# Tencent-RoboticsX/lifelike-agility-and-play

Measured on AMD Instinct MI355X. Metric: env-steps/sec (whole node), PMC tracking env, random policy, higher is better.
Workload: dtype f32

## Files before the change

### lifelike_agility_and_play_amd/csrc/llenv.hip

```cpp
#include <hip/hip_runtime.h>

#include <stdlib.h>

#include <new>
#include <type_traits>

#include "lanes.hpp"
#include "epmc_engine.hpp"
#include "sepmc_engine.hpp"
#include "pmc_engine.hpp"
#include "pmc_step.hpp"
#include "launch_plan.hpp"

#define HIPCHK(call)                                                                                   \
  do {                                                                                                 \
    hipError_t _e = (call);                                                                            \
    if (_e != hipSuccess) throw PmcError(LL_EHIP, std::string(#call) + ": " + hipGetErrorString(_e)); \
  } while (0)

typedef Pmc<GpuLanes> K;
typedef GpuLanesPinned<LC_COUNT> GpuLanes1;
#ifndef LL_PIN_EPMC
#define LL_PIN_EPMC 0
#endif
#ifndef LL_PIN_SEPMC
#define LL_PIN_SEPMC 0
#endif
#ifndef LL_PIN_PMC
#define LL_PIN_PMC 1
#endif
#ifndef LL_CONE_LDS
#define LL_CONE_LDS 1
#endif
#ifndef LL_CONE_LDS_SEPMC
#define LL_CONE_LDS_SEPMC 1
#endif
#ifndef LL_CONE_LDS_SEPMC1
#define LL_CONE_LDS_SEPMC1 1
#endif
#ifndef LL_PARK
#define LL_PARK 1
#endif
#ifndef LL_RELOAD_PMC
#define LL_RELOAD_PMC 1
#endif
#ifndef LL_RELOAD_EPMC1
#define LL_RELOAD_EPMC1 2
#endif
#ifndef LL_RELOAD_EPMC2
#define LL_RELOAD_EPMC2 1
#endif
#ifndef LL_SEPMC_RAY_CHUNK
#define LL_SEPMC_RAY_CHUNK 3
#endif
#ifndef LL_RELOAD_SEPMC2
#define LL_RELOAD_SEPMC2 1
#endif
#ifndef LL_SEPMC_ONE_WAVE_DEFAULT
#define LL_SEPMC_ONE_WAVE_DEFAULT 1
#endif
#ifndef LL_GRAM_PIPE_PMC1
#define LL_GRAM_PIPE_PMC1 0
#endif
typedef GpuLanesPinned<LC_COUNT, LL_PIN_PMC ? 7 : 0, LL_PIN_PMC ? BC_COUNT : 0, LL_PIN_PMC ? LK_BASE : 0> GpuLanesPmc1Plain;
typedef std::conditional<LL_GRAM_PIPE_PMC1 != 0, WithGramPipe<GpuLanesPmc1Plain>, GpuLanesPmc1Plain>::type GpuLanesPmc1;

__device__ __forceinline__ double wave_sum(double x) {
  for (int d = 32; d > 0; d >>= 1) x += __shfl_xor(x, d);
  return x;
}
__device__ __forceinline__ double ld_agent(const double* p) {
  return __builtin_bit_cast(double, __hip_atomic_load(reinterpret_cast<const unsigned long long*>(p), __ATOMIC_RELAXED, __HIP_MEMORY_SCOPE_AGENT));
}
__device__ __forceinline__ void st_agent(double* p, double v) {
  __hip_atomic_store(reinterpret_cast<unsigned long long*>(p), __builtin_bit_cast(unsigned long long, v), __ATOMIC_RELAXED, __HIP_MEMORY_SCOPE_AGENT);
}
__device__ __forceinline__ const StepParams& kernarg_params() {
  const __attribute__((address_space(4))) void* k = (const __attribute__((address_space(4))) void*)__builtin_amdgcn_kernarg_segment_ptr();
  asm volatile("" : "+s"(k));
  return *(const StepParams*)(const __attribute__((address_space(4))) StepParams*)k;
}
__device__ __forceinline__ void table_fold_wave(const StepParams& P, int sl, bool last_step) {
  const int lane = threadIdx.x & 63, n = P.n_clips;
  unsigned long long* pend_r = P.pending_reward + (long)sl * n;
  unsigned long long* pend_l = P.pending_len + (long)sl * n;
  const double* prev = sl == 0 ? P.cdf : P.cdf_ver + (long)sl * n;
  double* dst = last_step ? P.cdf : P.cdf_ver + (long)(sl + 1) * n;
  bool mine = false;
  for (int c = lane; c < n; c += PMC_WAVE) {
    const unsigned long long pr = __hip_atomic_load(pend_r + c, __ATOMIC_RELAXED, __HIP_MEMORY_SCOPE_AGENT);
    const unsigned long long pl = __hip_atomic_load(pend_l + c, __ATOMIC_RELAXED, __HIP_MEMORY_SCOPE_AGENT);
    if (pr) {
      st_agent(P.avg_reward + c, (double)__uint_as_float((uint32_t)pr));
      st_agent(P.avg_len + c, (double)__uint_as_float((uint32_t)pl));
      __hip_atomic_store(pend_r + c, 0ull, __ATOMIC_RELAXED, __HIP_MEMORY_SCOPE_AGENT);
      __hip_atomic_store(pend_l + c, 0ull, __ATOMIC_RELAXED, __HIP_MEMORY_SCOPE_AGENT);
      mine = true;
    }
  }
  if (!__any(mine)) {
    if (dst != prev) for (int c = lane; c < n; c += PMC_WAVE) st_agent(dst + c, ld_agent(prev + c));
    return;
  }
  asm volatile("s_waitcnt vmcnt(0)" ::: "memory");
  double part = 0.0;
  for (int c = lane; c < n; c += PMC_WAVE) {
    const double p = pow(1.0 - ld_agent(P.avg_reward + c), P.sample_factor);
    st_agent(P.prob + c, p);
    part += p;
  }
  asm volatile("s_waitcnt vmcnt(0)" ::: "memory");
  const double inv = 1.0 / wave_sum(part);
  double carry = 0.0;
  for (int c0 = 0; c0 < n; c0 += PMC_WAVE) {
    const int c = c0 + lane;
    double x = 0.0;
    if (c < n) { x = ld_agent(P.prob + c) * inv; st_agent(P.prob + c, x); }
    for (int d = 1; d < PMC_WAVE; d <<= 1) {
      const double y = __shfl_up(x, d);
      if (lane >= d) x += y;
    }
    x += carry;
    if (c < n) st_agent(dst + c, (c == n - 1) ? 1.0 : x);
    carry = __shfl(x, PMC_WAVE - 1);
  }
}
__device__ __attribute__((noinline)) void table_fold_wave_out_of_line(const StepParams& P, int sl, bool last_step) { table_fold_wave(P, sl, last_step); }
__device__ __forceinline__ void step_done_fold(const StepParams& P, int sl, bool last_step, bool multi) {
  asm volatile("s_waitcnt vmcnt(0)" ::: "memory");
  unsigned int ticket = 0;
  if (threadIdx.x == 0) ticket = __hip_atomic_fetch_add(P.block_ticket + sl, 1u, __ATOMIC_RELAXED, __HIP_MEMORY_SCOPE_AGENT);
  ticket = __builtin_amdgcn_readfirstlane(ticket);
  if (ticket != gridDim.x - 1) return;
  if (multi && sl > 0) {
    while (__hip_atomic_load(P.ver_ready + (sl - 1), __ATOMIC_RELAXED, __HIP_MEMORY_SCOPE_AGENT) != P.launch_serial) __builtin_amdgcn_s_sleep(2);
    LL_VER_FENCE(__ATOMIC_ACQUIRE);
  }
  asm volatile("" ::: "memory");
  if (multi) table_fold_wave_out_of_line(P, sl, last_step);
  else table_fold_wave(P, sl, last_step);
  if (threadIdx.x == 0) __hip_atomic_store(P.block_ticket + sl, 0u, __ATOMIC_RELAXED, __HIP_MEMORY_SCOPE_AGENT);
  if (multi) {
    asm volatile("s_waitcnt vmcnt(0)" ::: "memory");
    LL_VER_FENCE(__ATOMIC_RELEASE);
    if (threadIdx.x == 0) {
      __hip_atomic_store(P.ver_ready + sl, P.launch_serial, __ATOMIC_RELAXED, __HIP_MEMORY_SCOPE_AGENT);
      if (last_step) __hip_atomic_store(P.resident, 0u, __ATOMIC_RELAXED, __HIP_MEMORY_SCOPE_AGENT);
    }
  }
}

__device__ __forceinline__ float4 random_action_group(const StepParams& P, uint32_t gid, float sigma, int sl = 0) {
  uint32_t r[4];
  const uint64_t step = P.step_count + (uint64_t)sl;
  philox4x32(gid, (uint32_t)step, (uint32_t)(step >> 32), 0xAC710u, (uint32_t)P.seed, (uint32_t)(P.seed >> 32), r);
  const float k = 2.3283064365386963e-10f;
  float u1 = fminf(((float)r[0] + 1.0f) * k, 1.0f), u2 = (float)r[1] * k, u3 = fminf(((float)r[2] + 1.0f) * k, 1.0f), u4 = (float)r[3] * k;
  float m1 = sqrtf(-2.0f * logf(u1)), m2 = sqrtf(-2.0f * logf(u3));
  float4 o;
  o.x = sigma * m1 * cosf(6.283185307179586f * u2); o.y = sigma * m1 * sinf(6.283185307179586f * u2);
  o.z = sigma * m2 * cosf(6.283185307179586f * u4); o.w = sigma * m2 * sinf(6.283185307179586f * u4);
  return o;
}

template <class Lanes>
__device__ __forceinline__ void step_actions(const StepParams& P, const Lanes& ln, float* lds, int env, int sl, float* act) {
  if (P.action_sigma > 0.0f) {
    float* stash = lds + LC_COUNT * 4 + CAND_TABLE_WORDS * PMC_ROW + (threadIdx.x >> 4) * 12;
    const int l16 = threadIdx.x & 15;
    const uint32_t g = (uint32_t)(l16 < 3 ? l16 : 0);
    const float4 o = random_action_group(P, (uint32_t)env * 3u + g, P.action_sigma, sl);
    if (l16 < 3) {
      reinterpret_cast<float4*>(P.actions_out)[(long)env * 3 + l16] = o;
      reinterpret_cast<float4*>(stash)[l16] = o;
    }
    asm volatile("s_waitcnt lgkmcnt(0)" ::: "memory");
    for (int j = 0; j < 3; j++) act[j] = stash[ln.leg() * 3 + j];
  } else {
    for (int j = 0; j < 3; j++) act[j] = ln.ldl(P.actions, (long)env * 12 + j, 3);
  }
}

template <int OCC, bool OBST = false, bool MULTI = false, bool CONE = false, bool XROWS = false>
__global__ __launch_bounds__(PMC_WAVE, OCC) void pmc_step_kernel(StepParams P) {
  extern __shared__ __attribute__((aligned(16))) float lds[];
  const int env0 = blockIdx.x * PMC_ENVS_PER_WAVE + (threadIdx.x >> 4);
  typedef WithParamsReload<typename std::conditional<OCC == 1, GpuLanesPmc1, GpuLanes>::type, LL_RELOAD_PMC> Lanes0;
  typedef typename std::conditional<(OCC == 2 && CONE && LL_CONE_LDS), WithConeInLds<Lanes0>, Lanes0>::type Lanes;
  Lanes ln(lds);
  if constexpr (OCC == 1) ln.stage_consts(P.legc, LC_COUNT, P.candc, CAND_TABLE_WORDS, P.basec);
  else ln.stage_consts(P.legc, LC_COUNT, P.candc, CAND_TABLE_WORDS);
  if constexpr (!MULTI) {
    if (env0 < P.n_envs) {
      float act[3];
      step_actions(P, ln, lds, env0, 0, act);
      Pmc<Lanes>::template step_env<OBST, CONE, XROWS>(ln, P, env0, act, 0);
    }
    step_done_fold(P, 0, true, false);
  } else {
    if (threadIdx.x == 0) __hip_atomic_fetch_add(P.resident, 1u, __ATOMIC_RELAXED, __HIP_MEMORY_SCOPE_AGENT);
    for (int sl = 0; sl < P.n_steps; sl++) {
      if (sl) __builtin_amdgcn_fence(__ATOMIC_SEQ_CST, "workgroup");
      ln.new_step();
      int env = env0;
      asm volatile("" : "+v"(env));
      if (env < P.n_envs) {
        float act[3];
        PMC_PHASE("step.actions");
        step_actions(P, ln, lds, env, sl, act);
        Pmc<Lanes>::template step_env<OBST, CONE, XROWS>(ln, P, env, act, sl);
      }
      PMC_PHASE("step.table_fold");
      const StepParams& Pr = kernarg_params();
      step_done_fold(Pr, sl, sl == Pr.n_steps - 1, true);
    }
  }
}

template <int OCC, bool MULTI = false, bool CONE = false, bool XROWS = false>
__global__ __launch_bounds__(PMC_WAVE, OCC) void epmc_step_kernel(StepParams P, EpmcParams E) {
  extern __shared__ __attribute__((aligned(16))) float lds[];
  const int env0 = blockIdx.x * PMC_ENVS_PER_WAVE + (threadIdx.x >> 4);
  typedef WithRayChunk<WithShapePrefetch<WithParamsReload<typename std::conditional<OCC == 1 && LL_PIN_EPMC, GpuLanes1, GpuLanes>::type, (OCC == 1 ? LL_RELOAD_EPMC1 : LL_RELOAD_EPMC2)>, OCC == 2>, (OCC == 1 ? (MULTI ? 7 : 3) : 1)> Lanes0;
  typedef typename std::conditional<(OCC == 2 && CONE && LL_CONE_LDS), WithConeInLds<Lanes0>, Lanes0>::type Lanes;
  Lanes ln(lds);
  ln.stage_consts(P.legc, LC_COUNT, P.candc, CAND_TABLE_WORDS);
  if (env0 >= P.n_envs) return;
  if constexpr (!MULTI) {
    float act[3];
    step_actions(P, ln, lds, env0, 0, act);
    Epmc<Lanes>::template step_env<((OCC == 2 && LL_PARK) || LL_PARK > 1), CONE, XROWS>(ln, P, E, env0, act);
  } else {
    for (int sl = 0; sl < P.n_steps; sl++) {
      if (sl) __builtin_amdgcn_fence(__ATOMIC_SEQ_CST, "workgroup");
      ln.new_step();
      int env = env0;
      asm volatile("" : "+v"(env));
      float act[3];
      step_actions(P, ln, lds, env, sl, act);
      Epmc<Lanes>::template step_env<(LL_PARK > 1), CONE, XROWS>(ln, P, E, env, act);
    }
  }
}
__global__ __launch_bounds__(PMC_WAVE) void epmc_reset_kernel(StepParams P, EpmcParams E, const int32_t* ids, int n, const float* draws, const float* prev_orn) {
  extern __shared__ __attribute__((aligned(16))) float lds[];
  const int i = blockIdx.x * PMC_ENVS_PER_WAVE + (threadIdx.x >> 4);
  GpuLanes ln(lds);
  ln.stage_consts(P.legc, LC_COUNT, P.candc, CAND_TABLE_WORDS);
  if (i >= n) return;
  const int env = ids ? ids[i] : i;
  Epmc<GpuLanes>::reset_env(ln, P, E, env, draws ? draws + (long)i * EPMC_MAX_DRAWS : nullptr, prev_orn ? prev_orn + (long)i * 4 : nullptr);
}

#define PERCEPT_THREADS 128
__global__ __launch_bounds__(PERCEPT_THREADS) void epmc_percept_kernel(StepParams P, EpmcParams E) {
  __shared__ __attribute__((aligned(16))) float lists[3][EPMC_MAX_BOXES * EPMC_BOX_WORDS];
  __shared__ int cnt[3];
  const int row = blockIdx.x;
  const float* rec = E.ray_pose + (long)row * EPMC_RAY_POSE;
  if (threadIdx.x < 3) cnt[threadIdx.x] = 0;
  __syncthreads();
  typedef Epmc<GpuLanes> EP;
  const int nb = (int)rec[14];
  if ((int)threadIdx.x < nb) {
    M3<float> R;
    for (int i = 0; i < 9; i++) R.m[i] = rec[3 + i];
    const EP::RayBounds bd = EP::ray_bounds(rec, R);
    const BoxRec r = EP::ray_box(rec, E.boxes + (long)row * EPMC_MAX_BOXES * EPMC_BOX_WORDS, threadIdx.x);
    for (int fam = 0; fam < 3; fam++)
      if (EP::box_in_family(fam, r, rec, bd)) store_box(lists[fam] + atomicAdd(&cnt[fam], 1) * EPMC_BOX_WORDS, r);
  }
  __syncthreads();
  const float* lp[3] = {lists[0], lists[1], lists[2]};
  const int n[3] = {cnt[0], cnt[1], cnt[2]};
  EP::percept_rays(E, row, rec, lp, n, P.obs + (long)row * P.obs_dim + 3L * P.prop_dim + 36, threadIdx.x, PERCEPT_THREADS);
}

template <int OCC, bool MULTI = false, bool CONE = false, bool XROWS = false>
__global__ __launch_bounds__(PMC_WAVE, OCC) void sepmc_step_kernel(StepParams P, SepmcParams S) {
  extern __shared__ __attribute__((aligned(16))) float lds[];
  const int row0 = blockIdx.x * PMC_ENVS_PER_WAVE + (threadIdx.x >> 4);
  typedef typename std::conditional<OCC == 1 && LL_PIN_SEPMC, GpuLanes1, GpuLanes>::type PlainLanes;
  typedef WithRayChunk<WithShapePrefetch<typename std::conditional<(OCC == 2 && LL_RELOAD_SEPMC2), WithParamsReload<PlainLanes, LL_RELOAD_SEPMC2>, PlainLanes>::type, OCC == 1>, (OCC == 1 ? LL_SEPMC_RAY_CHUNK : 1)> Lanes0;
  typedef typename std::conditional<(CONE && ((OCC == 2 && LL_CONE_LDS_SEPMC) || (OCC == 1 && LL_CONE_LDS_SEPMC1))), WithConeInLds<Lanes0>, Lanes0>::type Lanes;
  Lanes ln(lds);
  ln.stage_consts(P.legc, LC_COUNT, P.candc, CAND_TABLE_WORDS);
  if (row0 >= P.n_envs) return;
  if constexpr (!MULTI) {
    float act[3];
    step_actions(P, ln, lds, row0, 0, act);
    Sepmc<Lanes>::template step_env<((OCC == 2 && LL_PARK) || LL_PARK > 1), CONE, XROWS>(ln, P, S, row0, act);
  } else {
    for (int sl = 0; sl < P.n_steps; sl++) {
      if (sl) __builtin_amdgcn_fence(__ATOMIC_SEQ_CST, "workgroup");
      ln.new_step();
      int row = row0;
      asm volatile("" : "+v"(row));
      float act[3];
      step_actions(P, ln, lds, row, sl, act);
      Sepmc<Lanes>::template step_env<(LL_PARK > 1), CONE, XROWS>(ln, P, S, row, act);
    }
  }
}
__global__ __launch_bounds__(PMC_WAVE) void sepmc_reset_kernel(StepParams P, SepmcParams S, const int32_t* ids, int n, const float* draws, const float* prev_orn) {
  extern __shared__ __attribute__((aligned(16))) float lds[];
  const int i = blockIdx.x * PMC_ENVS_PER_WAVE + (threadIdx.x >> 4);
  GpuLanes ln(lds);
  ln.stage_consts(P.legc, LC_COUNT, P.candc, CAND_TABLE_WORDS);
  if (i >= n) return;
  const int row = ids ? ids[i] : i;
  Sepmc<GpuLanes>::reset_env(ln, P, S, row, draws ? draws + (long)(i >> 1) * EPMC_MAX_DRAWS : nullptr, prev_orn ? prev_orn + (long)(i >> 1) * 4 : nullptr);
}

__global__ __launch_bounds__(PMC_WAVE) void pmc_reset_kernel(StepParams P, const int32_t* ids, int n, const int32_t* clip, const double* t0) {
  extern __shared__ __attribute__((aligned(16))) float lds[];
  const int i = blockIdx.x * PMC_ENVS_PER_WAVE + (threadIdx.x >> 4);
  GpuLanes ln(lds);
  ln.stage_consts(P.legc, LC_COUNT, P.candc, CAND_TABLE_WORDS);
  if (i >= n) return;
  const int env = ids ? ids[i] : i;
  int c;
  double t;
  uint32_t ep = P.ep_count[env] + 1;
  K::sample_start(ln, P, env, ep, &c, &t);
  P.ep_count[env] = ep;
  if (clip) c = clip[i];
  if (t0) t = t0[i];
  K::reset_env(ln, P, env, c, t);
  P.done[env] = 0;
  P.done_reason[env] = 0;
}

__global__ __launch_bounds__(PMC_WAVE) void pmc_probe_pd_kernel(StepParams P, const float* in, float* out, int n, int mode) {
  extern __shared__ __attribute__((aligned(16))) float lds[];
  const int i = blockIdx.x * PMC_ENVS_PER_WAVE + (threadIdx.x >> 4);
  GpuLanes ln(lds);
  ln.stage_consts(P.legc, LC_COUNT, P.candc, CAND_TABLE_WORDS);
  if (i >= n) return;
  K::probe_pd(ln, P, in + (long)i * 36, out + (long)i * 12, mode);
}

__global__ void pmc_gae_kernel(float* block, int n_envs, int unroll, int W, int od, float gamma, float lam, const float* bootstrap) {
  const int env = blockIdx.x * blockDim.x + threadIdx.x;
  if (env >= n_envs) return;
  float* rows = block + (size_t)env * unroll * W;
  float adv = 0.0f, vnext = bootstrap[env];
  for (int t = unroll - 1; t >= 0; t--) {
    float* r = rows + (size_t)t * W + od;
    const float V = r[14], m = r[16];
    const float delta = r[15] + gamma * vnext * m - V;
    adv = delta + gamma * lam * m * adv;
    r[13] = adv + V;
    vnext = V;
  }
}

__global__ void pmc_actions_kernel(StepParams P, float* actions, float sigma) {
  const int gid = blockIdx.x * blockDim.x + threadIdx.x;
  if (gid >= P.n_envs * 3) return;
  reinterpret_cast<float4*>(actions)[gid] = random_action_group(P, (uint32_t)gid, sigma);
}

#if defined(LL_KERNELS_ONLY)
template __global__ void LL_KERNELS_ONLY;
#else
struct HipBackend {
  int device;
  hipStream_t own = nullptr, stream = nullptr;
  bool timing = false;
  LaunchCaps caps;
  std::vector<std::pair<hipEvent_t, hipEvent_t>> evs;
  std::vector<int> ev_steps;
  size_t ev_used = 0;
  static constexpr size_t kMaxTimedLaunches = 16384;

  explicit HipBackend(int dev) : device(dev) {
    int n = 0;
    hipError_t e = hipGetDeviceCount(&n);
    if (e != hipSuccess || n <= 0) throw PmcError(LL_ENODEV, "no HIP device available: this engine has no CPU fallback");
    if (dev < 0 || dev >= n) throw PmcError(LL_EINVAL, "device ordinal out of range");
    HIPCHK(hipSetDevice(dev));
    HIPCHK(hipStreamCreateWithFlags(&own, hipStreamNonBlocking));
    hipDeviceProp_t prop;
    HIPCHK(hipGetDeviceProperties(&prop, dev));
    caps = launch_caps_from_env(prop.multiProcessorCount * 4, LL_SEPMC_ONE_WAVE_DEFAULT);
    stream = own;
  }
  ~HipBackend() {
    (void)hipSetDevice(device);
    for (auto& p : evs) { (void)hipEventDestroy(p.first); (void)hipEventDestroy(p.second); }
    if (own) (void)hipStreamDestroy(own);
  }
  void use() { HIPCHK(hipSetDevice(device)); }
  void set_stream(void* s) { stream = s ? (hipStream_t)s : own; }
  void* stream_handle() { return (void*)stream; }
  void* alloc(size_t bytes) {
    use();
    void* p = nullptr;
    HIPCHK(hipMalloc(&p, bytes ? bytes : 4));
    return p;
  }
  void release(void* p) { (void)hipSetDevice(device); (void)hipFree(p); }
  void zero(void* p, size_t bytes) { use(); HIPCHK(hipMemsetAsync(p, 0, bytes, stream)); }
  void h2d(void* d, const void* h, size_t bytes) {
    use();
    HIPCHK(hipMemcpyAsync(d, h, bytes, hipMemcpyHostToDevice, stream));
    HIPCHK(hipStreamSynchronize(stream));
  }
  void d2h(void* h, const void* d, size_t bytes) {
    use();
    HIPCHK(hipMemcpyAsync(h, d, bytes, hipMemcpyDeviceToHost, stream));
    HIPCHK(hipStreamSynchronize(stream));
  }
  void sync() { use(); HIPCHK(hipStreamSynchronize(stream)); }

  static size_t lds_bytes() { return ((size_t)LC_COUNT * 4 + (size_t)CAND_TABLE_WORDS * PMC_ROW + PMC_ENVS_PER_WAVE * 12) * sizeof(float); }
  static size_t lds_bytes_epmc() { return lds_bytes() + (size_t)PMC_ENVS_PER_WAVE * PMC_ROW_SCRATCH * sizeof(float); }
  static_assert(((size_t)LC_COUNT * 4 + (size_t)CAND_TABLE_WORDS * PMC_ROW + PMC_ENVS_PER_WAVE * 12 + (size_t)PMC_ENVS_PER_WAVE * PMC_ROW_SCRATCH) * sizeof(float) <= 160 * 1024 / 8,
                "eight single-wave workgroups per CU (two per SIMD) must fit the 160 KB of LDS");
  std::pair<hipEvent_t, hipEvent_t>* timing_begin(int n_steps = 1) {
    if (!timing) return nullptr;
    if (ev_used == kMaxTimedLaunches) return nullptr;
    if (ev_used == evs.size()) {
      hipEvent_t a, b;
      HIPCHK(hipEventCreate(&a));
      HIPCHK(hipEventCreate(&b));
      evs.push_back(std::make_pair(a, b));
      ev_steps.push_back(1);
    }
    ev_steps[ev_used] = n_steps;
    std::pair<hipEvent_t, hipEvent_t>* ev = &evs[ev_used++];
    HIPCHK(hipEventRecord(ev->first, stream));
    return ev;
  }
  void launch_percept(const StepParams& P, const EpmcParams& E) {
    hipLaunchKernelGGL(epmc_percept_kernel, dim3(P.n_envs), dim3(PERCEPT_THREADS), 0, stream, P, E);
  }
  template <class... Params> struct KernelTable {
    typedef void (*Kernel)(StepParams, Params...);
    Kernel at[StepBuild::kCount] = {};
    KernelTable(std::initializer_list<std::pair<StepBuild, Kernel>> builds) { for (const auto& e : builds) at[e.first.index()] = e.second; }
    Kernel operator[](const StepBuild& b) const {
      if (at[b.index()]) return at[b.index()];
      throw PmcError(LL_ESTATE, "the launch plan names a step-kernel build that is not compiled: (occ, obst, multi, cone, xrows) = (" + std::to_string(b.occ) + ", " + std::to_string(b.obst) + ", " + std::to_string(b.multi) + ", " + std::to_string(b.cone) + ", " + std::to_string(b.xrows) + ")");
    }
  };
#define LL_ARENA(KERNEL, OCC, MULTI, CONE, XROWS) {{OCC, false, MULTI, CONE, XROWS}, KERNEL<OCC, MULTI, CONE, XROWS>}
#define LL_ARENA_BUILDS(KERNEL)                                                                                                                                           \
  {LL_ARENA(KERNEL, 1, false, true, true),  LL_ARENA(KERNEL, 2, false, true, true),   LL_ARENA(KERNEL, 1, false, true, false), LL_ARENA(KERNEL, 1, false, false, false), \
   LL_ARENA(KERNEL, 2, false, true, false), LL_ARENA(KERNEL, 2, false, false, false), LL_ARENA(KERNEL, 1, true, true, false),  LL_ARENA(KERNEL, 1, true, false, false)}
  static inline const KernelTable<EpmcParams> epmc_kernels LL_ARENA_BUILDS(epmc_step_kernel);
  static inline const KernelTable<SepmcParams> sepmc_kernels LL_ARENA_BUILDS(sepmc_step_kernel);
#undef LL_ARENA_BUILDS
#undef LL_ARENA
#define LL_PMC(OCC, OBST, MULTI, CONE, XROWS) {{OCC, OBST, MULTI, CONE, XROWS}, pmc_step_kernel<OCC, OBST, MULTI, CONE, XROWS>}
  static inline const KernelTable<> pmc_kernels{
      LL_PMC(1, false, true, true, true),  LL_PMC(1, false, false, true, true),  LL_PMC(2, false, false, true, true),
      LL_PMC(1, true, true, true, false),  LL_PMC(1, true, false, true, false),  LL_PMC(2, true, true, true, false),  LL_PMC(2, true, false, true, false),
      LL_PMC(1, true, true, false, false), LL_PMC(1, true, false, false, false), LL_PMC(2, true, true, false, false), LL_PMC(2, true, false, false, false),
      LL_PMC(1, false, true, true, false), LL_PMC(1, false, false, true, false), LL_PMC(2, false, true, true, false), LL_PMC(2, false, false, true, false),
      LL_PMC(1, false, true, false, false), LL_PMC(1, false, false, false, false), LL_PMC(2, false, true, false, false), LL_PMC(2, false, false, false, false)};
#undef LL_PMC
  StepPlan plan(int engine, const StepParams& P, bool scripted_rays = false) const { return plan_step(engine, P, scripted_rays, caps); }
  static EpmcParams& rays_of(EpmcParams& E) { return E; } static EpmcParams& rays_of(SepmcParams& S) { return S.e; }
  template <class Params> void launch_arena_step(int engine, const KernelTable<Params>& kernels, const StepParams& P, const Params& X_in) {
    use();
    Params X = X_in;
    EpmcParams& E = rays_of(X);
    const StepPlan pl = plan(engine, P, E.scr_ray_hit != nullptr);
    const auto kernel = kernels[pl.build];
    std::pair<hipEvent_t, hipEvent_t>* ev = timing_begin(P.n_steps);
    E.split_rays = pl.percept ? 1 : 0;
    StepParams Q = P;
    Q.n_steps = pl.steps_per_launch;
    for (int done = 0; done < P.n_steps; done += Q.n_steps, Q.step_count += (uint64_t)Q.n_steps) {
      hipLaunchKernelGGL(kernel, dim3(pl.blocks), dim3(PMC_WAVE), lds_bytes_epmc(), stream, Q, X);
      if (pl.percept) launch_percept(Q, E);
    }
    HIPCHK(hipGetLastError());
    if (ev) HIPCHK(hipEventRecord(ev->second, stream));
  }
  void launch_epmc_step(const StepParams& P, const EpmcParams& E) { launch_arena_step(LL_ENGINE_EPMC, epmc_kernels, P, E); }
  void launch_epmc_reset(const StepParams& P, const EpmcParams& E, const int32_t* ids, int n, const float* draws, const float* prev_orn) {
    use();
    const int blocks = (n + PMC_ENVS_PER_WAVE - 1) / PMC_ENVS_PER_WAVE;
    hipLaunchKernelGGL(epmc_reset_kernel, dim3(blocks), dim3(PMC_WAVE), lds_bytes_epmc(), stream, P, E, ids, n, draws, prev_orn);
    HIPCHK(hipGetLastError());
  }
  void launch_sepmc_step(const StepParams& P, const SepmcParams& S) { launch_arena_step(LL_ENGINE_SEPMC, sepmc_kernels, P, S); }
  void launch_sepmc_reset(const StepParams& P, const SepmcParams& S, const int32_t* ids, int n, const float* draws, const float* prev_orn) {
    use();
    const int blocks = (n + PMC_ENVS_PER_WAVE - 1) / PMC_ENVS_PER_WAVE;
    hipLaunchKernelGGL(sepmc_reset_kernel, dim3(blocks), dim3(PMC_WAVE), lds_bytes_epmc(), stream, P, S, ids, n, draws, prev_orn);
    HIPCHK(hipGetLastError());
  }
  void launch_step(const StepParams& P) {
    use();
    const StepPlan pl = plan(LL_ENGINE_PMC, P);
    if (P.n_steps > pl.steps_per_launch) throw PmcError(LL_ESTATE, "a launch of " + std::to_string(P.n_steps) + " control steps where the launch plan carries at most " + std::to_string(pl.steps_per_launch));
    const auto kernel = pmc_kernels[pl.build];
    std::pair<hipEvent_t, hipEvent_t>* ev = timing_begin(P.n_steps);
    hipLaunchKernelGGL(kernel, dim3(pl.blocks), dim3(PMC_WAVE), pl.row_scratch ? lds_bytes_epmc() : lds_bytes(), stream, P);
    HIPCHK(hipGetLastError());
    if (ev) HIPCHK(hipEventRecord(ev->second, stream));
  }
  void launch_reset(const StepParams& P, const int32_t* ids, int n, const int32_t* clip, const double* t0) {
    use();
    const int blocks = (n + PMC_ENVS_PER_WAVE - 1) / PMC_ENVS_PER_WAVE;
    hipLaunchKernelGGL(pmc_reset_kernel, dim3(blocks), dim3(PMC_WAVE), lds_bytes(), stream, P, ids, n, clip, t0);
    HIPCHK(hipGetLastError());
  }
  void launch_probe_pd(const StepParams& P, const float* in, float* out, int n, int mode) {
    use();
    hipLaunchKernelGGL(pmc_probe_pd_kernel, dim3((n + PMC_ENVS_PER_WAVE - 1) / PMC_ENVS_PER_WAVE), dim3(PMC_WAVE), lds_bytes(), stream, P, in, out, n, mode);
    HIPCHK(hipGetLastError());
  }
  void launch_gae(float* block, int n_envs, int unroll, int W, int od, float gamma, float lam, const float* bootstrap) {
    use();
    hipLaunchKernelGGL(pmc_gae_kernel, dim3((n_envs + 255) / 256), dim3(256), 0, stream, block, n_envs, unroll, W, od, gamma, lam, bootstrap);
    HIPCHK(hipGetLastError());
  }
  void launch_actions(const StepParams& P, float* actions, float sigma) {
    use();
    const int threads = 256;
    hipLaunchKernelGGL(pmc_actions_kernel, dim3((P.n_envs * 3 + threads - 1) / threads), dim3(threads), 0, stream, P, actions, sigma);
    HIPCHK(hipGetLastError());
  }
  void enable_timing(bool on) { timing = on; }
  void collect_timing(double* avg_ms, int* n, long long* n_steps = nullptr) {
    sync();
    double tot = 0;
    long long steps = 0;
    for (size_t i = 0; i < ev_used; i++) {
      float ms = 0;
      HIPCHK(hipEventElapsedTime(&ms, evs[i].first, evs[i].second));
      tot += ms;
      steps += ev_steps[i];
    }
    *n = (int)ev_used;
    *avg_ms = ev_used ? tot / ev_used : 0.0;
    if (n_steps) *n_steps = steps;
    ev_used = 0;
  }
};

typedef PmcEngine<HipBackend> ENGINE;
#include "pmc_capi.inc"
typedef EpmcEngine<HipBackend> EPMC_ENGINE;
#include "epmc_capi.inc"
typedef SepmcEngine<HipBackend> SEPMC_ENGINE;
#include "sepmc_capi.inc"
#include "pmc_policy.inc"
#include "hl_policy.inc"
#include "hl_unroll.inc"
#include "hl_league.inc"
#include "xfer_capi.inc"
#endif
```

### lifelike_agility_and_play_amd/csrc/pmc_params.hpp

```cpp
#pragma once
#include <stdint.h>

#define LL_UNROLL_EXTRA 17
#define PMC_K 4
#define PMC_WAVE 64
#define PMC_ENVS_PER_WAVE 4

enum LegConst {
  LC_R1 = 0,
  LC_R2 = 3,
  LC_R3 = 6,
  LC_M = 9,
  LC_COM = 12,
  LC_IC = 21,
  LC_QLO = 39,
  LC_QHI = 42,
  LC_JDAMP = 45,
  LC_FOOT = 48,
  LC_BSX = 51,
  LC_BSY = 52,
  LC_HANDLE = 53,
  LC_HAS_HANDLE = 57,
  LC_HIPCYL = 58,
  LC_THBOX = 69,
  LC_THCYL0 = 81,
  LC_THCYL1 = 92,
  LC_WHEEL = 103,
  LC_SHBOX = 114,
  LC_FOOTSPH = 126,
  LC_CAPS = 130,
  LC_TRUNKCAP = 144,
  LC_COUNT = 151
};

enum CandField { CF_A = 0, CF_AX = 3, CF_FB = 6, CF_R = 9, CF_LINK = 10, CF_KIND = 11, CF_WORDS = 12 };
#define CAND_PER_SUB 8
#define LK_BASE (CAND_PER_SUB * CF_WORDS)
#define LK_WORDS 10
#define CAND_TABLE_WORDS (CAND_PER_SUB * CF_WORDS + LK_WORDS)

enum BaseConst {
  BC_MASS = 0,
  BC_H = 1,
  BC_IO = 4,
  BC_COM = 10,
  BC_ICOM = 13,
  BC_BOX = 19,
  BC_COUNT = 31
};

#if defined(PMC_ABLATION)
#define PMC_ABL(bit) ((P.debug_flags & (bit)) != 0)
#define PMC_TS_SLOTS 32
#define PMC_TS(k) do { if (PMC_ABL(16) && ln.is_lane(0)) P.counters[4 + (long)env * PMC_TS_SLOTS + (k)] = wall_clock64(); } while (0)
#else
#define PMC_ABL(bit) false
#define PMC_TS_SLOTS 0
#define PMC_TS(k) do { } while (0)
#endif
#ifndef LL_VER_FENCES
#define LL_VER_FENCES 1
#endif
#if LL_VER_FENCES && defined(__HIP_DEVICE_COMPILE__)
#define LL_VER_FENCE(order) __builtin_amdgcn_fence(order, "agent")
#else
#define LL_VER_FENCE(order) do { } while (0)
#endif

#if defined(PMC_MARKS) && defined(__HIP_DEVICE_COMPILE__)
#define PMC_PHASE(name) do { __builtin_amdgcn_sched_barrier(0); asm volatile("; LLPHASE " name ::: "memory"); __builtin_amdgcn_sched_barrier(0); } while (0)
#else
#define PMC_PHASE(name) do { } while (0)
#endif

#ifndef PMC_PGS_HOIST
#define PMC_PGS_HOIST 1
#endif

#ifndef PMC_PGS_HOIST_PAIR
#define PMC_PGS_HOIST_PAIR 1
#endif
#ifndef PMC_PGS_HOIST_TERRAIN
#define PMC_PGS_HOIST_TERRAIN 0
#endif

#define LL_MAX_STEPS_PER_LAUNCH 128

struct StepParams {
  static constexpr bool kFirstKernelArgument = true;
  int32_t n_envs, n_sub, n_iter, auto_reset;
  int32_t n_clips, prop_dim, obs_dim, frame_rate;
  int32_t margin, envs_per_wave;
  int32_t prop_off[5];
  int32_t keep_term_obs;
  float dt, kp, kd, max_tau;
  float max_tau1, pad6;
  float mu_foot, mu_link, gravity, link_damping;
  float erp, margin_dist, limit_gate, self_collision;
  float rw[5];
  float max_depen;
  float self_margin;
  int32_t friction_dirs;
  int32_t friction_mode;
  float limit_erp;
  float erp_deep, limit_erp_deep, erp_deep_below;
  float spec_erp_deep, spec_limit_erp, spec_limit_erp_deep;
  int32_t limit_speculative;
  float max_coord_vel;
  int32_t max_contacts, max_self;
  float self_friction, pair_friction;
  int32_t max_pair, leg_edges;
  double dt_d, frame_step, policy_step, sample_factor;
  uint64_t seed;
  uint64_t step_count;

  float* state;
  float* kin;
  float* feet;
  double* time;
  int32_t* clip;
  int32_t* ep_steps;
  float* reward_sum;
  uint32_t* ep_count;
  float* obs;
  float* term_obs;
  float* reward;
  uint8_t* done;
  uint8_t* done_reason;
  const float* actions;
  const float* scripted_state;
  const float* scripted_feet;
  float* traj;
  int32_t traj_slot, traj_buf, traj_unroll, traj_nbuf;
  const float* neglogp;
  const float* value;
  const double* frames;
  const int32_t* clip_off;
  const int32_t* clip_len;
  const double* max_steps;
  double* cdf;
  double* prob;
  double* avg_reward;
  double* avg_len;
  unsigned int* block_ticket;
  double* cdf_ver;
  unsigned int* ver_ready;
  unsigned int* resident;
  uint32_t launch_serial;
  int32_t table_versions;
  float* actions_out;
  float action_sigma;
  int32_t n_steps;
  const int32_t* ob_off;
  const int32_t* ob_cnt;
  const double* ob_table;
  int32_t* ob_id;
  float ob_half_height, ob_pad;
  int32_t set_obstacle, debug_flags;
  unsigned long long* pending_reward;
  unsigned long long* pending_len;
  unsigned long long* counters;
  unsigned long long* ep_hist;
  const float* legc;
  const float* candc;
  const float* basec;
};

LL_HD bool pmc_wants_xrows(const StepParams& P) { return P.self_friction > 0.0f || P.pair_friction > 0.0f || P.max_pair != LLM_MAX_PAIR; }
LL_HD bool pmc_wants_xrows_terrain(const StepParams& P) { return pmc_wants_xrows(P) || P.leg_edges != 0; }
```

Measured before the change: 21.58 million.

## Overlap next-step action sampling with grid ticket fold and add single-wave fold path

```diff
diff --git a/lifelike_agility_and_play_amd/csrc/llenv.hip b/lifelike_agility_and_play_amd/csrc/llenv.hip
--- a/lifelike_agility_and_play_amd/csrc/llenv.hip
+++ b/lifelike_agility_and_play_amd/csrc/llenv.hip
@@ -86,6 +86,41 @@
   unsigned long long* pend_l = P.pending_len + (long)sl * n;
   const double* prev = sl == 0 ? P.cdf : P.cdf_ver + (long)sl * n;
   double* dst = last_step ? P.cdf : P.cdf_ver + (long)(sl + 1) * n;
+  if (n <= PMC_WAVE) {
+    const bool in = lane < n;
+    unsigned long long pr = 0ull, pl = 0ull;
+    double avg = 0.0;
+    if (in) {
+      pr = __hip_atomic_load(pend_r + lane, __ATOMIC_RELAXED, __HIP_MEMORY_SCOPE_AGENT);
+      pl = __hip_atomic_load(pend_l + lane, __ATOMIC_RELAXED, __HIP_MEMORY_SCOPE_AGENT);
+      avg = ld_agent(P.avg_reward + lane);
+    }
+    if (!__any(pr != 0ull)) {
+      if (dst != prev && in) st_agent(dst + lane, ld_agent(prev + lane));
+      return;
+    }
+    if (pr) {
+      avg = (double)__uint_as_float((uint32_t)pr);
+      st_agent(P.avg_reward + lane, avg);
+      st_agent(P.avg_len + lane, (double)__uint_as_float((uint32_t)pl));
+      __hip_atomic_store(pend_r + lane, 0ull, __ATOMIC_RELAXED, __HIP_MEMORY_SCOPE_AGENT);
+      __hip_atomic_store(pend_l + lane, 0ull, __ATOMIC_RELAXED, __HIP_MEMORY_SCOPE_AGENT);
+    }
+    double p = 0.0, part = 0.0;
+    if (in) {
+      p = pow(1.0 - avg, P.sample_factor);
+      part += p;
+    }
+    const double inv = 1.0 / wave_sum(part);
+    double x = 0.0;
+    if (in) { x = p * inv; st_agent(P.prob + lane, x); }
+    for (int d = 1; d < PMC_WAVE; d <<= 1) {
+      const double y = __shfl_up(x, d);
+      if (lane >= d) x += y;
+    }
+    if (in) st_agent(dst + lane, (lane == n - 1) ? 1.0 : x);
+    return;
+  }
   bool mine = false;
   for (int c = lane; c < n; c += PMC_WAVE) {
     const unsigned long long pr = __hip_atomic_load(pend_r + c, __ATOMIC_RELAXED, __HIP_MEMORY_SCOPE_AGENT);
@@ -126,17 +161,28 @@
   }
 }
 __device__ __attribute__((noinline)) void table_fold_wave_out_of_line(const StepParams& P, int sl, bool last_step) { table_fold_wave(P, sl, last_step); }
-__device__ __forceinline__ void step_done_fold(const StepParams& P, int sl, bool last_step, bool multi) {
+struct NoStamp { __device__ void operator()(int) const {} };
+template <class Stamp = NoStamp>
+__device__ __forceinline__ unsigned int step_take_ticket(const StepParams& P, int sl, const Stamp& stamp = Stamp()) {
   asm volatile("s_waitcnt vmcnt(0)" ::: "memory");
+  stamp(33);
+  long lane_zero = 0;
+  asm volatile("" : "+v"(lane_zero));
   unsigned int ticket = 0;
-  if (threadIdx.x == 0) ticket = __hip_atomic_fetch_add(P.block_ticket + sl, 1u, __ATOMIC_RELAXED, __HIP_MEMORY_SCOPE_AGENT);
+  if (threadIdx.x == 0) ticket = __hip_atomic_fetch_add(P.block_ticket + sl + lane_zero, 1u, __ATOMIC_RELAXED, __HIP_MEMORY_SCOPE_AGENT);
+  return ticket;
+}
+template <class Stamp = NoStamp>
+__device__ __forceinline__ void step_fold_if_last(const StepParams& P, int sl, bool last_step, bool multi, unsigned int ticket, const Stamp& stamp = Stamp()) {
   ticket = __builtin_amdgcn_readfirstlane(ticket);
+  stamp(34);
   if (ticket != gridDim.x - 1) return;
   if (multi && sl > 0) {
     while (__hip_atomic_load(P.ver_ready + (sl - 1), __ATOMIC_RELAXED, __HIP_MEMORY_SCOPE_AGENT) != P.launch_serial) __builtin_amdgcn_s_sleep(2);
     LL_VER_FENCE(__ATOMIC_ACQUIRE);
   }
   asm volatile("" ::: "memory");
+  stamp(35);
   if (multi) table_fold_wave_out_of_line(P, sl, last_step);
   else table_fold_wave(P, sl, last_step);
   if (threadIdx.x == 0) __hip_atomic_store(P.block_ticket + sl, 0u, __ATOMIC_RELAXED, __HIP_MEMORY_SCOPE_AGENT);
@@ -148,6 +194,10 @@
       if (last_step) __hip_atomic_store(P.resident, 0u, __ATOMIC_RELAXED, __HIP_MEMORY_SCOPE_AGENT);
     }
   }
+  stamp(36);
+}
+__device__ __forceinline__ void step_done_fold(const StepParams& P, int sl, bool last_step, bool multi) {
+  step_fold_if_last(P, sl, last_step, multi, step_take_ticket(P, sl));
 }
 
 __device__ __forceinline__ float4 random_action_group(const StepParams& P, uint32_t gid, float sigma, int sl = 0) {
@@ -163,6 +213,36 @@
   return o;
 }
 
+__device__ __forceinline__ float draw_action(const StepParams& P, int env, int sl) {
+  if (!(P.action_sigma > 0.0f)) return 0.0f;
+  const int l16 = threadIdx.x & 15, j = l16 & 3;
+  const uint32_t g = (uint32_t)(l16 < 12 ? l16 >> 2 : 0);
+  uint32_t r[4];
+  const uint64_t step = P.step_count + (uint64_t)sl;
+  philox4x32((uint32_t)env * 3u + g, (uint32_t)step, (uint32_t)(step >> 32), 0xAC710u, (uint32_t)P.seed, (uint32_t)(P.seed >> 32), r);
+  const float k = 2.3283064365386963e-10f;
+  const uint32_t ra = (j & 2) ? r[2] : r[0], rb = (j & 2) ? r[3] : r[1];
+  const float u1 = fminf(((float)ra + 1.0f) * k, 1.0f), u2 = (float)rb * k;
+  const float m = sqrtf(-2.0f * logf(u1));
+  const float a = 6.283185307179586f * u2;
+  const float trig = (j & 1) ? sinf(a) : cosf(a);
+  return P.action_sigma * m * trig;
+}
+template <class Lanes>
+__device__ __forceinline__ void take_actions(const StepParams& P, const Lanes& ln, float* lds, int env, float drawn, float* act) {
+  if (P.action_sigma > 0.0f) {
+    float* stash = lds + LC_COUNT * 4 + CAND_TABLE_WORDS * PMC_ROW + (threadIdx.x >> 4) * 12;
+    const int l16 = threadIdx.x & 15;
+    if (l16 < 12) {
+      P.actions_out[(long)env * 12 + l16] = drawn;
+      stash[l16] = drawn;
+    }
+    asm volatile("s_waitcnt lgkmcnt(0)" ::: "memory");
+    for (int j = 0; j < 3; j++) act[j] = stash[ln.leg() * 3 + j];
+  } else {
+    for (int j = 0; j < 3; j++) act[j] = ln.ldl(P.actions, (long)env * 12 + j, 3);
+  }
+}
 template <class Lanes>
 __device__ __forceinline__ void step_actions(const StepParams& P, const Lanes& ln, float* lds, int env, int sl, float* act) {
   if (P.action_sigma > 0.0f) {
@@ -193,26 +273,43 @@
   if constexpr (!MULTI) {
     if (env0 < P.n_envs) {
       float act[3];
-      step_actions(P, ln, lds, env0, 0, act);
+      take_actions(P, ln, lds, env0, draw_action(P, env0, 0), act);
       Pmc<Lanes>::template step_env<OBST, CONE, XROWS>(ln, P, env0, act, 0);
     }
     step_done_fold(P, 0, true, false);
   } else {
     if (threadIdx.x == 0) __hip_atomic_fetch_add(P.resident, 1u, __ATOMIC_RELAXED, __HIP_MEMORY_SCOPE_AGENT);
+    float drawn = 0.0f;
+    if (env0 < P.n_envs) drawn = draw_action(P, env0, 0);
     for (int sl = 0; sl < P.n_steps; sl++) {
-      if (sl) __builtin_amdgcn_fence(__ATOMIC_SEQ_CST, "workgroup");
       ln.new_step();
       int env = env0;
       asm volatile("" : "+v"(env));
-      if (env < P.n_envs) {
+      const bool on = env < P.n_envs;
+      const bool ts = on && sl == P.n_steps - 2;
+      (void)ts;
+      auto stamp = [&](int k) { if (ts) PMC_TS(k); };
+      if (on) {
         float act[3];
-        PMC_PHASE("step.actions");
-        step_actions(P, ln, lds, env, sl, act);
+        take_actions(P, ln, lds, env, drawn, act);
         Pmc<Lanes>::template step_env<OBST, CONE, XROWS>(ln, P, env, act, sl);
       }
+      stamp(32);
       PMC_PHASE("step.table_fold");
       const StepParams& Pr = kernarg_params();
-      step_done_fold(Pr, sl, sl == Pr.n_steps - 1, true);
+      if (sl == Pr.n_steps - 1) step_done_fold(Pr, sl, true, true);
+      else {
+        asm volatile("s_waitcnt vmcnt(0)" ::: "memory");
+        __builtin_amdgcn_fence(__ATOMIC_SEQ_CST, "workgroup");
+        const unsigned int ticket = step_take_ticket(Pr, sl, stamp);
+        PMC_PHASE("step.actions");
+        if (on) drawn = draw_action(Pr, env, sl + 1);
+        asm volatile("" : "+v"(drawn));
+        const unsigned long long t_drawn = PMC_TS_NOW();
+        PMC_PHASE("step.table_fold");
+        step_fold_if_last(Pr, sl, false, true, ticket, stamp);
+        if (ts) PMC_TS_AT(37, t_drawn);
+      }
     }
   }
 }
diff --git a/lifelike_agility_and_play_amd/csrc/pmc_params.hpp b/lifelike_agility_and_play_amd/csrc/pmc_params.hpp
--- a/lifelike_agility_and_play_amd/csrc/pmc_params.hpp
+++ b/lifelike_agility_and_play_amd/csrc/pmc_params.hpp
@@ -51,12 +51,16 @@
 
 #if defined(PMC_ABLATION)
 #define PMC_ABL(bit) ((P.debug_flags & (bit)) != 0)
-#define PMC_TS_SLOTS 32
+#define PMC_TS_SLOTS 40
 #define PMC_TS(k) do { if (PMC_ABL(16) && ln.is_lane(0)) P.counters[4 + (long)env * PMC_TS_SLOTS + (k)] = wall_clock64(); } while (0)
+#define PMC_TS_NOW() wall_clock64()
+#define PMC_TS_AT(k, t) do { if (PMC_ABL(16) && ln.is_lane(0)) P.counters[4 + (long)env * PMC_TS_SLOTS + (k)] = (t); } while (0)
 #else
 #define PMC_ABL(bit) false
 #define PMC_TS_SLOTS 0
 #define PMC_TS(k) do { } while (0)
+#define PMC_TS_NOW() 0ull
+#define PMC_TS_AT(k, t) do { (void)(t); } while (0)
 #endif
 #ifndef LL_VER_FENCES
 #define LL_VER_FENCES 1
```

New measurement: 21.71 million (median of 6 runs). About the same (+0.6%).
